# FernandoSchett/parallel_finite_difference_computation

Hardware: AMD Instinct MI355X
Metric: Gpoints/s (stencil updates) + achieved HBM GB/s vs peak (higher is better)
Workload: dtype f32

## Files before the change

include/fdwave.h:

```cpp
#ifndef FDWAVE_H
#define FDWAVE_H

#include <stddef.h>

#ifdef __cplusplus
extern "C" {
#endif

#define FDW_VERSION 2
#define FDW_MAX_ORDER 32

#define FDW_OK 0
#define FDW_EINVAL (-1)
#define FDW_ENODEVICE (-2)
#define FDW_EHIP (-3)
#define FDW_ENOMEM (-4)
#define FDW_ESTATE (-5)
#define FDW_ECOMM (-6)

typedef struct fdw_ctx fdw_ctx;

typedef struct fdw_params {
    int order;
    int nxe, nze;
// ... 212 lines not shown
int fdw_image_unscale_v2(const float *v2, int nxe, int nze, int nxb, int nzb, int nx, int nz, const float *img , float *out);
int fdw_shot_dtt(fdw_ctx *ctx, const float *v2 , int sx, int sz, int gz, const float *srce, const float *d_obs, float *imloc,
                 float *illum , int residual , float *resid , float *P, float *PP);
int fdw_shot_line_dtt(fdw_ctx *ctx, const float *v2, int sz, int gz, const float *wav, const float *d_obs, float *imloc, float *illum, int residual,
                      float *resid, float *P, float *PP);
int fdw_shot_batch_dtt(fdw_ctx *ctx, int nshots, const float *v2_all, unsigned long long draw_offset, int sx0, int dsx, int sz, int gz,
                       const float *srce, const float *d_obs, float *imloc, float *illum, int residual, float *resid);
int fdw_shot_line_batch_dtt(fdw_ctx *ctx, int nshots, const float *v2_all, unsigned long long draw_offset, int sz, int gz, const float *wav_all,
                            const float *d_obs, float *imloc, float *illum, int residual, float *resid);

int fdw_set_tuning(fdw_ctx *ctx, int xchunk, int wz, int use_generic, int prefetch, int two_step);
int fdw_get_tables(const fdw_ctx *ctx, float *coefs_x, float *coefs_z, float *taper_x, float *taper_z);
int fdw_get_extents(const fdw_ctx *ctx, int *xlim, int *zlim, int *ztap);
int fdw_debug_step4_plan(fdw_ctx *ctx, int forward, int sx, int sz, int r0, int r1, int r0b, int r1b, int xchunk, int *nblk, int *nstrip,
                         unsigned char *cls, int cls_cap);
int fdw_two_step_active(const fdw_ctx *ctx);
int fdw_steps_per_pass(const fdw_ctx *ctx);
int fdw_selftest(fdw_ctx *ctx);
int fdw_trace_active(void);

#define FDW_PASS_DEPTH_MAX 3
typedef struct fdw_band_unit {
    int pass, band;
    int r0, r1;
    int stream;
    int nwait;
    int wait[FDW_PASS_DEPTH_MAX - 1];
} fdw_band_unit;
int fdw_plan_pass_bands(int nxl, int upd_x1, int xchunk, int bands, int depth, int npasses, int *bands_out, int *depth_out,
                        fdw_band_unit *units, int cap);
int fdw_set_pass_bands(fdw_ctx *ctx, int bands, int depth);
int fdw_pass_bands(const fdw_ctx *ctx, int *bands, int *depth);

int fdw_calc_coefs(int order, int cxx, float *coef );
void fdw_ricker_wavelet(int nt, float dt, float fpeak, float *s);
void fdw_taper_tables(int nxb, int nzb, float fac, float *taper_x, float *taper_z);
void fdw_extendvel_linear(int nx, int nz, int nxb, int nzb, float *vel);
void fdw_srand(unsigned seed);

#ifdef __cplusplus
}
#endif
#endif
```

parallel_finite_difference_computation_amd/__init__.py:

```python
from ._lib import BORN_DTT, BORN_FIELD, IMAGE_DTT, IMAGE_XCORR, FdwError, LIB_PATH, MODE_FWD, MODE_PLAIN, MODE_RECV, lib
from .api import (FDWave, calc_coefs, extendvel_linear, fd_back, fd_forward, fd_init, image_compare, gather_misfit, gather_scale_v2, image_unscale_v2, image_compensate, image_excitation, image_laplacian, mod_extendvel,
                  mod_ricker_wavelet, mod_taper_tables, ricker_wavelet, snap_dims, srand, taper_tables, planewave_lags, encode_line_source, encode_gathers, encode_gathers_multi, plan_pass_bands)

from .slabs import Comm, Slabs, run_ranks

__all__ = ["Comm", "Slabs", "run_ranks", "FDWave", "FdwError", "calc_coefs", "ricker_wavelet", "taper_tables", "extendvel_linear", "srand",
           "fd_init", "fd_forward", "fd_back", "mod_extendvel", "mod_ricker_wavelet", "mod_taper_tables", "image_laplacian", "image_compare", "image_compensate", "image_excitation", "gather_misfit", "snap_dims", "planewave_lags", "encode_line_source", "encode_gathers", "encode_gathers_multi", "plan_pass_bands", "lib", "LIB_PATH", "MODE_FWD", "MODE_PLAIN", "MODE_RECV", "BORN_FIELD", "BORN_DTT", "IMAGE_XCORR", "IMAGE_DTT", "gather_scale_v2", "image_unscale_v2"]
```

parallel_finite_difference_computation_amd/_lib.py:

```python
import ctypes as C
import os

import numpy as np

_HERE = os.path.dirname(os.path.abspath(__file__))
LIB_PATH = os.environ.get("FDW_LIB") or os.path.join(_HERE, "libfdwave.so")

f32p = np.ctypeslib.ndpointer(dtype=np.float32, flags="C_CONTIGUOUS")
vp = C.c_void_p

FDW_OK, FDW_EINVAL, FDW_ENODEVICE, FDW_EHIP, FDW_ENOMEM, FDW_ESTATE = 0, -1, -2, -3, -4, -5
MODE_FWD, MODE_PLAIN, MODE_RECV = 0, 1, 2
BORN_FIELD, BORN_DTT = 0, 1
IMAGE_XCORR, IMAGE_DTT = 0, 1


class FdwError(RuntimeError):
    def __init__(self, code, msg):
        super().__init__(f"libfdwave error {code}: {msg}")
        self.code = code


class Params(C.Structure):
    _fields_ = [("order", C.c_int), ("nxe", C.c_int), ("nze", C.c_int), ("nxb", C.c_int), ("nzb", C.c_int),
# ... 122 lines not shown
    ("fdw_dev_line_record_illum_steps", C.c_int, [vp, C.POINTER(vp), vp, vp, C.c_int, C.c_int, vp, vp, C.c_int, C.c_int, C.c_int, C.POINTER(C.c_int), C.POINTER(C.c_int), vp]),
    ("fdw_shot_line_residual", C.c_int, [vp, vp, C.c_int, C.c_int, f32p, f32p, f32p, vp, vp, vp, vp]),
    ("fdw_shot_line_batch", C.c_int, [vp, C.c_int, vp, C.c_ulonglong, C.c_int, C.c_int, f32p, f32p, f32p, vp]),
    ("fdw_shot_line_batch_residual", C.c_int, [vp, C.c_int, vp, C.c_ulonglong, C.c_int, C.c_int, f32p, f32p, f32p, vp, vp]),
    ("fdw_record_shot_line_batch", C.c_int, [vp, C.c_int, vp, C.c_ulonglong, C.c_int, C.c_int, f32p, f32p]),
    ("fdw_encode_gathers_multi", C.c_int, [C.c_int, C.c_int, C.c_int, vp, vp, vp, C.c_int, C.c_int, vp]),
    ("fdw_dev_excite_steps", C.c_int, [vp, C.POINTER(vp), vp, vp, C.c_int, C.c_int, vp, vp, C.c_int, C.c_int, C.c_int, C.POINTER(C.c_int), C.POINTER(C.c_int), vp]),
    ("fdw_dev_line_pick_steps", C.c_int, [vp, C.POINTER(vp), vp, vp, C.c_int, vp, C.c_int, vp, C.c_int, C.c_int, C.c_int, C.POINTER(C.c_int), C.POINTER(C.c_int), vp]),
    ("fdw_shot_excitation", C.c_int, [vp, vp, C.c_int, C.c_int, C.c_int, vp, vp, C.c_float, vp, vp, vp, vp, vp, vp]),
    ("fdw_image_excitation", C.c_int, [vp, vp, C.c_size_t, C.c_float, vp]),
    ("fdw_dev_image_excitation", C.c_int, [vp, vp, vp, C.c_float, vp, vp]),
    ("fdw_shot_excitation_batch", C.c_int, [vp, C.c_int, vp, C.c_ulonglong, C.c_int, C.c_int, C.c_int, C.c_int, vp, vp, C.c_float, vp, vp, vp, vp, vp]),
    ("fdw_dev_born_steps", C.c_int, [vp, vp, vp, vp, vp, vp, vp, C.c_int, vp, C.c_int, C.c_int, C.c_int, vp, vp, C.c_int, C.c_int, C.c_int, vp]),
    ("fdw_born_shot", C.c_int, [vp, vp, f32p, C.c_int, C.c_int, C.c_int, C.c_int, f32p, f32p, vp]),
    ("fdw_dev_born_line_steps", C.c_int, [vp, vp, vp, vp, vp, vp, vp, C.c_int, vp, C.c_int, C.c_int, vp, vp, C.c_int, C.c_int, C.c_int, vp]),
    ("fdw_born_shot_line", C.c_int, [vp, vp, vp, C.c_int, C.c_int, C.c_int, vp, vp, vp]),
    ("fdw_born_shot_batch", C.c_int, [vp, C.c_int, vp, C.c_ulonglong, vp, C.c_int, C.c_int, C.c_int, C.c_int, C.c_int, vp, vp, vp]),
    ("fdw_born_shot_line_batch", C.c_int, [vp, C.c_int, vp, C.c_ulonglong, vp, C.c_int, C.c_int, C.c_int, vp, vp, vp]),
    ("fdw_dev_back_iter_dtt", C.c_int, [vp, C.c_int, vp, vp, vp, vp, vp, C.c_int, C.c_int, C.c_int, vp, C.c_int, vp, vp]),
    ("fdw_dev_dtt_image", C.c_int, [vp, vp, vp, vp, vp, vp, vp]),
    ("fdw_gather_scale_v2", C.c_int, [f32p, C.c_int, C.c_int, C.c_int, C.c_int, C.c_int, C.c_int, f32p, f32p]),
    ("fdw_image_unscale_v2", C.c_int, [f32p, C.c_int, C.c_int, C.c_int, C.c_int, C.c_int, C.c_int, f32p, f32p]),
    ("fdw_shot_dtt", C.c_int, [vp, vp, C.c_int, C.c_int, C.c_int, f32p, f32p, f32p, vp, C.c_int, vp, vp, vp]),
    ("fdw_shot_line_dtt", C.c_int, [vp, vp, C.c_int, C.c_int, f32p, f32p, f32p, vp, C.c_int, vp, vp, vp]),
    ("fdw_shot_batch_dtt", C.c_int, [vp, C.c_int, vp, C.c_ulonglong, C.c_int, C.c_int, C.c_int, C.c_int, f32p, f32p, f32p, vp, C.c_int, vp]),
    ("fdw_shot_line_batch_dtt", C.c_int, [vp, C.c_int, vp, C.c_ulonglong, C.c_int, C.c_int, f32p, f32p, f32p, vp, C.c_int, vp]),
    ("fdw_two_step_active", C.c_int, [vp]),
    ("fdw_steps_per_pass", C.c_int, [vp]),
    ("fdw_selftest", C.c_int, [vp]),
    ("fdw_trace_active", C.c_int, []),
    ("fdw_plan_pass_bands", C.c_int, [C.c_int] * 6 + [C.POINTER(C.c_int)] * 2 + [vp, C.c_int]),
    ("fdw_set_pass_bands", C.c_int, [vp, C.c_int, C.c_int]),
    ("fdw_pass_bands", C.c_int, [vp, C.POINTER(C.c_int), C.POINTER(C.c_int)]),
    ("fdw_calc_coefs", C.c_int, [C.c_int, C.c_int, f32p]),
    ("fdw_ricker_wavelet", None, [C.c_int, C.c_float, C.c_float, f32p]),
    ("fdw_taper_tables", None, [C.c_int, C.c_int, C.c_float, vp, vp]),
    ("fdw_extendvel_linear", None, [C.c_int, C.c_int, C.c_int, C.c_int, f32p]),
    ("fdw_srand", None, [C.c_uint]),
]

_lib = None


def lib():
    global _lib
    if _lib is None:
        if not os.path.exists(LIB_PATH):
            raise ImportError(f"{LIB_PATH} is missing: build it with `make -C {os.path.join(_HERE, 'csrc')}` "
                              "(hipcc, gfx950).  There is no CPU fallback.")
        L = C.CDLL(LIB_PATH, mode=C.RTLD_GLOBAL)
        for name, res, args in SIGNATURES:
            fn = getattr(L, name)
            fn.restype = res
            fn.argtypes = args
        _lib = L
    return _lib


def check(rc):
    if rc != 0:
        raise FdwError(rc, lib().fdw_last_error().decode(errors="replace"))
```

parallel_finite_difference_computation_amd/api.py:

```python
import ctypes as C
import sys

import numpy as np

from . import _lib
from ._lib import Params, Slab, Snaps, check, lib


def _f32(a, shape=None):
    a = np.ascontiguousarray(a, dtype=np.float32)
    if shape is not None and a.shape != tuple(shape):
        raise ValueError(f"expected shape {tuple(shape)}, got {a.shape}")
    return a


def calc_coefs(order, cxx=False):
    c = np.zeros(order + 1, np.float32)
    check(lib().fdw_calc_coefs(order, int(cxx), c))
    return c


def ricker_wavelet(nt, dt, fpeak):
    s = np.zeros(nt, np.float32)
    lib().fdw_ricker_wavelet(nt, dt, fpeak, s)
# ... 79 lines not shown

def gather_scale_v2(v2, nxb, gz, g):
    v2, g = np.ascontiguousarray(v2, np.float32), np.ascontiguousarray(g, np.float32)
    out = np.empty_like(g)
    check(lib().fdw_gather_scale_v2(v2, v2.shape[0], v2.shape[1], int(nxb), int(gz), g.shape[0], g.shape[1], g, out))
    return out


def image_unscale_v2(v2, nxb, nzb, img):
    v2, img = np.ascontiguousarray(v2, np.float32), np.ascontiguousarray(img, np.float32)
    out = np.empty_like(img)
    check(lib().fdw_image_unscale_v2(v2, v2.shape[0], v2.shape[1], int(nxb), int(nzb), img.shape[0], img.shape[1], img, out))
    return out


def snap_dims(nx, nz, nt, every, dec=1):
    a, b, c = C.c_int(), C.c_int(), C.c_int()
    check(lib().fdw_snap_dims(nx, nz, nt, int(every), int(dec), C.byref(a), C.byref(b), C.byref(c)))
    return a.value, b.value, c.value


def _i32(a):
    return np.ascontiguousarray(a, dtype=np.int32).reshape(-1)


def plan_pass_bands(nxl, upd_x1, xchunk, bands, depth, npasses):
    g, d = C.c_int(), C.c_int()
    n = lib().fdw_plan_pass_bands(nxl, upd_x1, xchunk, bands, depth, npasses, C.byref(g), C.byref(d), None, 0)
    check(min(n, 0))
    units = (_lib.BandUnit * n)()
    check(min(lib().fdw_plan_pass_bands(nxl, upd_x1, xchunk, bands, depth, npasses, C.byref(g), C.byref(d), units, n), 0))
    return g.value, d.value, [dict(pass_=u.pass_, band=u.band, r0=u.r0, r1=u.r1, stream=u.stream, wait=[u.wait[k] for k in range(u.nwait)])
                              for u in units]


def planewave_lags(src_ix, dx, dt, p):
    src_ix = _i32(src_ix)
    lag = np.zeros(src_ix.size, np.int32)
    check(lib().fdw_planewave_lags(src_ix.size, src_ix.ctypes.data, dx, dt, float(p), lag.ctypes.data))
    return lag


def encode_line_source(src_ix, lag, weight, srce, nx):
    src_ix, lag, weight, srce = _i32(src_ix), _i32(lag), _f32(weight).reshape(-1), _f32(srce).reshape(-1)
    if not (src_ix.size == lag.size == weight.size):
        raise ValueError("src_ix, lag and weight must have one entry per shot")
    wav = np.zeros((nx, srce.size), np.float32)
    check(lib().fdw_encode_line_source(src_ix.size, src_ix.ctypes.data, lag.ctypes.data, weight.ctypes.data, srce.ctypes.data, srce.size, nx,
                                       wav.ctypes.data))
    return wav


def encode_gathers(lag, weight, d_obs_all, device=0):
    lag, weight = _i32(lag), _f32(weight).reshape(-1)
    d_obs_all = np.ascontiguousarray(d_obs_all, np.float32)
    if d_obs_all.ndim != 3 or not (d_obs_all.shape[0] == lag.size == weight.size):
        raise ValueError("d_obs_all must be [nshots][nx][nt] with one lag and one weight per shot")
    _, nx, nt = d_obs_all.shape
    out = np.zeros((nx, nt), np.float32)
    check(lib().fdw_encode_gathers(device, lag.size, lag.ctypes.data, weight.ctypes.data, d_obs_all.ctypes.data, nx, nt, out.ctypes.data))
    return out


def encode_gathers_multi(lag, weight, d_obs_all, device=0):
    lag, weight = np.ascontiguousarray(lag, np.int32), _f32(weight)
    d_obs_all = np.ascontiguousarray(d_obs_all, np.float32)
# ... 36 lines not shown
            self.close()
        except Exception:
            pass

    def tables(self):
        cx = np.zeros(self.order + 1, np.float32)
        cz = np.zeros(self.order + 1, np.float32)
        tx = np.zeros(max(self.nxb, 1), np.float32)
        tz = np.zeros(max(self.nzb, 1), np.float32)
        check(lib().fdw_get_tables(self._h, cx.ctypes.data, cz.ctypes.data, tx.ctypes.data, tz.ctypes.data))
        return cx, cz, tx[:self.nxb], tz[:self.nzb]

    def extents(self):
        a, b, c = C.c_int(), C.c_int(), C.c_int()
        check(lib().fdw_get_extents(self._h, C.byref(a), C.byref(b), C.byref(c)))
        return a.value, b.value, c.value

    def set_tuning(self, xchunk=0, wz=0, use_generic=False, prefetch=0, two_step=0, force_edge=False):
        check(lib().fdw_set_tuning(self._h, xchunk, wz, int(use_generic), prefetch, int(two_step)))

    def two_step_active(self):
        return bool(lib().fdw_two_step_active(self._h))

    def steps_per_pass(self):
        return int(lib().fdw_steps_per_pass(self._h))

    def set_pass_bands(self, bands=0, depth=0):
        check(lib().fdw_set_pass_bands(self._h, int(bands), int(depth)))

    def pass_bands(self):
        a, b = C.c_int(), C.c_int()
        check(lib().fdw_pass_bands(self._h, C.byref(a), C.byref(b)))
        return a.value, b.value

    def selftest(self):
        check(lib().fdw_selftest(self._h))

    def laplacian(self, p):
        p = _f32(p, (self.nxe, self.nze))
        out = np.empty_like(p)
        check(lib().fdw_laplacian(self._h, p, out))
        return out

    def forward(self, v2, sx, sz, srce, p=None, pp=None, nsteps=None):
        shape = (self.nxe, self.nze)
        p = np.zeros(shape, np.float32) if p is None else np.array(p, np.float32, order="C")
        pp = np.zeros(shape, np.float32) if pp is None else np.array(pp, np.float32, order="C")
        srce = _f32(srce)
        nsteps = len(srce) if nsteps is None else nsteps
        if nsteps > len(srce):
            raise ValueError("srce shorter than nsteps")
        check(lib().fdw_forward(self._h, p, pp, _f32(v2, shape), sx, sz, srce, nsteps))
        return p, pp

    def back(self, v2, snap0, snap1, d_obs, gz, imloc=None, nsteps=None):
        shape = (self.nxe, self.nze)
        imloc = np.zeros((self.nx, self.nz), np.float32) if imloc is None else np.array(imloc, np.float32, order="C")
        nsteps = self.nt if nsteps is None else nsteps
        check(lib().fdw_back(self._h, _f32(v2, shape), _f32(snap0, shape), _f32(snap1, shape),
                             _f32(d_obs, (self.nx, self.nt)), gz, imloc, nsteps))
        return imloc

    def shot(self, v2, sx, sz, gz, srce, d_obs, imloc=None, want_fields=False, want_illum=False, illum=None):
        shape = (self.nxe, self.nze)
        imloc = np.zeros((self.nx, self.nz), np.float32) if imloc is None else np.array(imloc, np.float32, order="C")
        P = np.zeros(shape, np.float32) if want_fields else None
# ... 500 lines not shown
```

parallel_finite_difference_computation_amd/csrc/fdw_api.cpp:

```cpp
#include <hip/hip_runtime.h>

#include <algorithm>
#include <climits>
#include <cmath>
#include <cstdarg>
#include <cstdio>
#include <cstdlib>
#include <cstring>
#include <mutex>
#include <new>
#include <type_traits>
#include <vector>

#include "fdw_born.h"
#include "fdw_dtt.h"
#include "fdw_excimg.h"
#include "fdw_internal.h"
#include "fdw_kernels.h"
#include "fdwave.h"

using namespace fdw;

static thread_local char g_err[512] = "";

// ... 54 lines not shown
    int nbatch = 1, batch_dsx = 0, batch_cap = 0, batch_nt = 0;
    bool batch_all = false;
    float* bfld[8] = {nullptr, nullptr, nullptr, nullptr, nullptr, nullptr, nullptr, nullptr};
    float *b_v2 = nullptr, *b_img = nullptr, *b_dobs = nullptr;
    float* b_illum = nullptr;
    int b_illum_cap = 0;
    bool batch_illum = false;
    float* b_rec = nullptr;
    size_t b_rec_cap = 0;
    float* d_wav = nullptr;
    size_t wav_cap = 0;
    float* b_wav = nullptr;
    size_t b_wav_cap = 0;
    float* d_raw = nullptr;
    size_t raw_cap = 0;
    int no_fused_back = 0;
    int no_back_pipe = 0;
    int no_back_fused = 0;
    int no_born_fused = 0;
    float* d_born_m = nullptr;
    float* d_born_rec0 = nullptr;
    size_t born_rec0_cap = 0;
    float* d_dtt_w = nullptr;
    float* d_born_w = nullptr;
    float* b_born_rec0 = nullptr;
    size_t b_born_rec0_cap = 0;
    size_t store_budget = 0;
    int store_segments = 0;
    size_t batch_budget = 0;
    int batch_parts = 0;
    bool batch_single = false;
    int pb_bands = 0, pb_depth = 0;
    int pb_used_bands = 0, pb_used_depth = 0;
    hipStream_t pb_side[FDW_PASS_DEPTH_MAX - 1] = {};
    hipEvent_t pb_fork = nullptr, pb_join[FDW_PASS_DEPTH_MAX - 1] = {}, pb_ring[kBandRing] = {};
};

static size_t field_elems(const fdw_ctx* c) { return (size_t)c->nxl * (size_t)c->pitch; }

extern "C" int fdw_pitch(const fdw_ctx* c) { return c ? c->pitch : 0; }
extern "C" size_t fdw_field_bytes(const fdw_ctx* c) { return c ? field_elems(c) * sizeof(float) : 0; }

static int is_full_grid(const fdw_ctx* c) { return c->slab.x_off == 0 && c->nxl == c->prm.nxe; }

static hipStream_t pick_stream(fdw_ctx* c, void* s) { return s ? (hipStream_t)s : c->stream; }

static int alloc_zero(float** p, size_t elems)
{
    if (*p) return FDW_OK;
    hipError_t e = hipMalloc((void**)p, elems * sizeof(float));
    if (e != hipSuccess) return fail(FDW_ENOMEM, "hipMalloc(%zu bytes) failed: %s", elems * sizeof(float), hipGetErrorString(e));
    HIP_TRY(hipMemset(*p, 0, elems * sizeof(float)));
    HIP_TRY(hipDeviceSynchronize());
    return FDW_OK;
}

static int ensure_work_buffers(fdw_ctx* c, int nfields, bool need_img)
{
    for (int i = 0; i < nfields; i++) {
        int rc = alloc_zero(&c->fld[i], field_elems(c));
        if (rc) return rc;
    }
    int rc = alloc_zero(&c->d_v2, field_elems(c));
    if (rc) return rc;
    if (need_img) {
        rc = alloc_zero(&c->d_img, field_elems(c));
// ... 710 lines not shown
    if (c->tb == kPipeSteps) return true;
    if (c->tb > 0) return false;
    return (long)c->upd_x1 * ((c->pitch / 4 + 55) / 56) >= kPipeAutoStripRows;
}

struct StepnBack {
    float *lvl0 = nullptr, *lvl1 = nullptr;
    const float* plev[kPipeSteps] = {};
    float* img = nullptr;
    int inj_stride = 0;
    const float *rp = nullptr, *rpp = nullptr;
    float *rout1 = nullptr, *rout2 = nullptr;
};
static void tile_classes(const Step2Args& a, const FwdVariant& v, std::vector<unsigned char>& cls)
{
    constexpr int H = kMaxFastHalfOrder, NS = kPipeSteps;
    cls.resize((size_t)a.nblk);
    for (int L = 0; L < a.nblk; L++) {
        FDW_PIPE_TILE_ROWS(a, L, zb, xa, xe)
        const int cs = FDW_PIPE_TILE_CELL(zb, NS);
        const bool lean = v.kmode == FDW_MODE_PLAIN ? pipe_tile_lean<H, NS, false, 0>(a, cs, xa, xe)
                          : (v.line && v.rec)       ? pipe_tile_lean<H, NS, true, 2, false, true>(a, cs, xa, xe)
                          : v.line                  ? pipe_tile_lean<H, NS, true, 2>(a, cs, xa, xe)
                                                    : pipe_tile_lean<H, NS, true, 1>(a, cs, xa, xe);
        cls[(size_t)L] = lean ? 0 : 1;
    }
}

static int pipe_strips(const fdw_ctx* c)
{
    const int ncells = c->pitch / 4, own = 64 - 2 * kPipeSteps;
    return (ncells + own - 1) / own;
}
static int pipe_fwd_xchunk(const fdw_ctx* c, long strip_rows)
{
    const bool fastnum = c->prm.numerics == FDW_NUMERICS_FAST;
    return c->xchunk2 > 0 ? c->xchunk2 : (strip_rows >= 1000000 ? 253 : (strip_rows >= 250000 ? 173 : (strip_rows >= 120000 ? (fastnum ? 173 : 143) : (strip_rows >= 60000 ? 83 : 43))));
}

struct StepnPlan {
    int nblk = 0, nstrip = 0;
    std::vector<unsigned char> cls;
};
static thread_local StepnPlan* g_plan = nullptr;

static int stepn_impl(fdw_ctx* c, int mode, const float* d_p, const float* d_pp, const float* d_v2, float* d_out1, float* d_out2, int pp_twice,
                      const FwdView& f, const StepnBack& bk, const RowRanges& rr, hipStream_t s)
{
    const bool recv = mode == FDW_MODE_RECV || mode == FDW_MODE_BACK4;
    if (c->h != kMaxFastHalfOrder) return fail(FDW_EINVAL, "stepn: the pipelined kernel is built for order 8 only");
    if (mode != FDW_MODE_FWD && mode != FDW_MODE_PLAIN && mode != FDW_MODE_MOD && mode != FDW_MODE_PLAIN_ALL && mode != FDW_MODE_RECV && mode != FDW_MODE_BACK4)
        return fail(FDW_EINVAL, "stepn: FWD, PLAIN, PLAIN_ALL, RECV, BACK4 or MOD only");
    if (mode == FDW_MODE_BACK4) {
        if (!bk.img || !f.samples || !bk.rp || !bk.rpp || !bk.rout1 || !bk.rout2) return fail(FDW_EINVAL, "stepn: BACK4 needs the receiver pair, its outputs, samples and image");
        const float* all[8] = {d_p, d_pp, d_out1, d_out2, bk.rp, bk.rpp, bk.rout1, bk.rout2};
        for (int i = 0; i < 8; i++)
            for (int j = i + 1; j < 8; j++)
                if (all[i] == all[j]) return fail(FDW_EINVAL, "stepn: BACK4 buffers must not alias");
    }
    if ((mode == FDW_MODE_PLAIN_ALL && (!bk.lvl0 || !bk.lvl1)) ||
        (mode == FDW_MODE_RECV && (!bk.img || !f.samples || !bk.plev[0] || !bk.plev[1] || !bk.plev[2] || !bk.plev[3])))
        return fail(FDW_EINVAL, "stepn: the backward passes need their level buffers / source fields, samples and image");
    if ((mode == FDW_MODE_MOD) != (c->prm.dialect == FDW_DIALECT_MOD)) return fail(FDW_ESTATE, "stepn: mode %d does not belong to dialect %d", mode, c->prm.dialect);
    if (!d_p || !d_pp || !d_v2 || !d_out1 || !d_out2) return fail(FDW_EINVAL, "stepn: NULL buffer");
    if (d_out1 == d_p || d_out1 == d_pp || d_out2 == d_p || d_out2 == d_pp || d_out1 == d_out2)
        return fail(FDW_EINVAL, "stepn: outputs must not alias the inputs (tiles re-read each other's input rows)");
    Step2Args a{};
    fill_common(c, a, d_p, d_pp, d_v2, pp_twice);
    a.out1 = d_out1; a.out2 = d_out2;
// ... 172 lines not shown
    if (npasses > INT_MAX / G) return fail(FDW_EINVAL, "pass bands: %d passes of %d bands", npasses, G);
    if (bands_out) *bands_out = G;
    if (depth_out) *depth_out = D;
    const int total = G * npasses;
    for (int i = 0; units && i < std::min(cap, total); i++) {
        fdw_band_unit& u = units[i];
        u.pass = i / G; u.band = i % G;
        u.r0 = G == 1 ? 0 : first_chunk(u.band) * xchunk;
        u.r1 = u.band == G - 1 ? nxl : first_chunk(u.band + 1) * xchunk;
        u.stream = i % D;
        u.nwait = 0;
        for (int k = 0; k < FDW_PASS_DEPTH_MAX - 1; k++) u.wait[k] = -1;
        for (int j = i - D - 1; j >= i - 2 * D + 1 && j >= 0; j--) u.wait[u.nwait++] = j;
    }
    return total;
}

extern "C" int fdw_set_pass_bands(fdw_ctx* c, int bands, int depth)
{
    if (!c) return fail(FDW_EINVAL, "ctx is NULL");
    if (bands < 0 || depth < 0 || depth > FDW_PASS_DEPTH_MAX || (bands == 0) != (depth == 0))
        return fail(FDW_EINVAL, "pass bands: bands=%d depth=%d (0, 0 = automatic; depth 1..%d)", bands, depth, FDW_PASS_DEPTH_MAX);
    c->pb_bands = bands; c->pb_depth = depth;
    return FDW_OK;
}

extern "C" int fdw_pass_bands(const fdw_ctx* c, int* bands, int* depth)
{
    if (!c || !bands || !depth) return fail(FDW_EINVAL, "NULL argument");
    *bands = c->pb_used_bands; *depth = c->pb_used_depth;
    return FDW_OK;
}

constexpr int kBandAutoTiles = 1776, kBandAutoPasses = 8;
static void wanted_pass_bands(const fdw_ctx* c, long tiles, int npasses, int* bands, int* depth)
{
    *bands = *depth = 1;
    if (c->pb_bands > 0) {
        *bands = c->pb_bands; *depth = c->pb_depth;
    } else if (const char* e = getenv("FDW_PASS_BANDS")) {
        int g = 0, d = 0;
        if (sscanf(e, "%d,%d", &g, &d) == 2 && g >= 1 && d >= 1 && d <= FDW_PASS_DEPTH_MAX) { *bands = g; *depth = d; }
    } else if (tiles >= kBandAutoTiles && npasses >= kBandAutoPasses) {
        *bands = 3; *depth = 2;
    }
}

static int ensure_band_streams(fdw_ctx* c, int depth)
{
    if (!c->pb_fork) HIP_TRY(hipEventCreateWithFlags(&c->pb_fork, hipEventDisableTiming));
    for (hipEvent_t& e : c->pb_ring)
        if (!e) HIP_TRY(hipEventCreateWithFlags(&e, hipEventDisableTiming));
    for (int j = 0; j < depth - 1; j++) {
        if (!c->pb_side[j]) HIP_TRY(hipStreamCreateWithFlags(&c->pb_side[j], hipStreamNonBlocking));
        if (!c->pb_join[j]) HIP_TRY(hipEventCreateWithFlags(&c->pb_join[j], hipEventDisableTiming));
    }
    return FDW_OK;
}

static int band_passes(fdw_ctx* c, float* const* buf, const float* d_v2, const Forward& f, int it0, int npasses, int first_pp_twice, int* ip, int* ipp,
                       hipStream_t s, int G, int D, int xchunk)
{
    std::vector<fdw_band_unit> units((size_t)G * npasses);
    int g_ = 0, d_ = 0;
    const int total = fdw_plan_pass_bands(c->nxl, c->upd_x1, xchunk, G, D, npasses, &g_, &d_, units.data(), (int)units.size());
    if (total < 0) return total;
    if (g_ != G || d_ != D || total != (int)units.size()) return fail(FDW_ESTATE, "pass bands: the plan changed between two calls");
    hipStream_t st[FDW_PASS_DEPTH_MAX] = {s};
    if (D > 1) {
        FDW_TRY(ensure_band_streams(c, D));
        HIP_TRY(hipEventRecord(c->pb_fork, s));
        for (int j = 1; j < D; j++) {
            st[j] = c->pb_side[j - 1];
            HIP_TRY(hipStreamWaitEvent(st[j], c->pb_fork, 0));
        }
    }
    auto issue = [&]() -> int {
        int o1 = 0, o2 = 0;
        for (int i = 0; i < total; i++) {
            const fdw_band_unit& u = units[(size_t)i];
            if (u.band == 0) spare_pair(*ip, *ipp, &o1, &o2);
            const int k = u.pass * kPipeSteps;
            for (int w = 0; w < u.nwait; w++) HIP_TRY(hipStreamWaitEvent(st[u.stream], c->pb_ring[u.wait[w] % kBandRing], 0));
            FDW_TRY(stepn_impl(c, FDW_MODE_FWD, buf[*ipp], buf[*ip], d_v2, buf[o1], buf[o2], (k > 0) || first_pp_twice, view_at(f, it0 + k, c->nx), StepnBack{},
                                RowRanges{u.r0, u.r1, 0, 0, xchunk}, st[u.stream]));
            if (D > 1 && i + D + 1 < total) HIP_TRY(hipEventRecord(c->pb_ring[i % kBandRing], st[u.stream]));
            if (u.band == G - 1) { *ip = o1; *ipp = o2; }
        }
        return FDW_OK;
    };
    const int rc = issue();
    char msg[sizeof g_err];
    if (rc != FDW_OK) memcpy(msg, g_err, sizeof msg);
    int jrc = FDW_OK;
    for (int j = 1; j < D; j++) {
        hipError_t e = hipEventRecord(c->pb_join[j - 1], st[j]);
        if (e == hipSuccess) e = hipStreamWaitEvent(s, c->pb_join[j - 1], 0);
        if (e != hipSuccess && jrc == FDW_OK) jrc = fail(FDW_EHIP, "pass bands: joining side stream %d failed: %s", j, hipGetErrorString(e));
    }
    if (rc != FDW_OK) memcpy(g_err, msg, sizeof msg);
    return rc != FDW_OK ? rc : jrc;
}

static int single_steps_on_copies(fdw_ctx* c, float* const* buf, const float* d_v2, const Forward& f, int it, int m, int twice, int ip, int ipp, int o1,
                                  int o2, hipStream_t s)
{
    const size_t bytes = field_elems(c) * sizeof(float) * (size_t)std::max(c->nbatch, 1);
    const float* newest = buf[ipp];
    for (int j = 0; j < m; j++) {
        float* dst = buf[(j & 1) ? o2 : o1];
        if (j < 2) HIP_TRY(hipMemcpyAsync(dst, buf[j == 0 ? ip : ipp], bytes, hipMemcpyDeviceToDevice, s));
        FDW_TRY(step_impl(c, FDW_MODE_FWD, newest, dst, d_v2, 0, c->nxl, twice || j > 0, view_at(f, it + j, c->nx), BackExtra{}, s));
        newest = dst;
    }
    return FDW_OK;
}

static int steps_loop(fdw_ctx* c, float* const* buf, const float* d_v2, const Forward& f, int it0, int nsteps, int first_pp_twice, int* ip, int* ipp,
                      hipStream_t s)
{
    if (!c || !buf || !ip || !ipp) return fail(FDW_EINVAL, "NULL argument");
    if (*ip < 0 || *ip > 3 || *ipp < 0 || *ipp > 3 || *ip == *ipp) return fail(FDW_EINVAL, "steps2: bad buffer indices");
    const FwdVariant var = fwd_variant(FDW_MODE_FWD, f);
    if (var.kmode < 0) return fail(FDW_EINVAL, "steps: no kernel is built for this combination of a line source, recording, illumination and excitation");
    if (f.rec) FDW_TRY(record_static(c, buf[*ip], buf[*ipp], f.gz, f.rec, it0, nsteps, s));
    int k = 0;
    c->pb_used_bands = c->pb_used_depth = 1;
    if (f.may_band && var.kmode == FDW_MODE_FWD && c->nbatch <= 1 && nsteps >= kPipeSteps && pipe_pays(c)) {
        const int nstrip = pipe_strips(c), xchunk = pipe_fwd_xchunk(c, (long)c->upd_x1 * nstrip), npasses = nsteps / kPipeSteps;
        int G, D;
        wanted_pass_bands(c, (long)nstrip * ((c->upd_x1 + xchunk - 1) / xchunk), npasses, &G, &D);
        if (G > 1 && fdw_plan_pass_bands(c->nxl, c->upd_x1, xchunk, G, D, npasses, &G, &D, nullptr, 0) < 0) return FDW_EINVAL;
        if (G > 1) {
            c->pb_used_bands = G; c->pb_used_depth = D;
            FDW_TRY(band_passes(c, buf, d_v2, f, it0, npasses, first_pp_twice, ip, ipp, s, G, D, xchunk));
            k = npasses * kPipeSteps;
        }
    }
    while (k < nsteps) {
        const int twice = (k > 0) || first_pp_twice;
        const FwdView v = view_at(f, it0 + k, c->nx);
        const int m = (nsteps - k >= kPipeSteps && pipe_pays(c)) ? kPipeSteps : ((nsteps - k >= 2 && two_step_pays(c)) ? 2 : 1);
        if (m == 1) {
            std::swap(*ip, *ipp);
            FDW_TRY(step_impl(c, FDW_MODE_FWD, buf[*ip], buf[*ipp], d_v2, 0, c->nxl, twice, v, BackExtra{}, s));
            k += 1;
            continue;
        }
        int o1, o2;
        spare_pair(*ip, *ipp, &o1, &o2);
        if (!family_serves(m, var))
            FDW_TRY(single_steps_on_copies(c, buf, d_v2, f, it0 + k, m, twice, *ip, *ipp, o1, o2, s));
        else if (m == kPipeSteps)
            FDW_TRY(stepn_impl(c, FDW_MODE_FWD, buf[*ipp], buf[*ip], d_v2, buf[o1], buf[o2], twice, v, StepnBack{}, RowRanges{}, s));
        else
            FDW_TRY(step2_impl(c, FDW_MODE_FWD, buf[*ipp], buf[*ip], d_v2, buf[o1], buf[o2], twice, v, BackExtra{}, s));
        *ip = o1; *ipp = o2;
        k += m;
    }
    return FDW_OK;
}

extern "C" int fdw_dev_steps2(fdw_ctx* c, float* const* buf, const float* d_v2, const float* d_srce, int sx, int sz, int it0, int nsteps,
                              int first_pp_twice, int* ip, int* ipp, void* stream)
{
// ... 2176 lines not shown
```

Before: 721.0.

## Add moving-cut two-stream pass schedule for temporally blocked forward steps

Adds a pass scheduler that splits each multi-step pass at a cut column which sweeps back and forth between lo and hi chunks. The two halves run on two streams with event waits only where halo reach overlaps, so consecutive passes can overlap and tail underutilisation is hidden. A three-piece turn handles direction reversals, and medium-sized grids get a different x-chunk size (213). The band executor is generalised into unit_passes, which records events only for units that are actually awaited. The cost is more event and stream synchronisation and a more complex dependency plan.

```diff
diff --git a/include/fdwave.h b/include/fdwave.h
--- a/include/fdwave.h
+++ b/include/fdwave.h
@@ -268,6 +268,11 @@
 int fdw_set_pass_bands(fdw_ctx *ctx, int bands, int depth);
 int fdw_pass_bands(const fdw_ctx *ctx, int *bands, int *depth);
 
+int fdw_plan_pass_cut(int nxl, int upd_x1, int xchunk, int cut_lo, int cut_hi, int npasses, int *lo_out, int *hi_out, fdw_band_unit *units,
+                      int cap);
+int fdw_set_pass_cut(fdw_ctx *ctx, int lo, int hi);
+int fdw_pass_cut(const fdw_ctx *ctx, int *lo, int *hi, int *turns);
+
 int fdw_calc_coefs(int order, int cxx, float *coef );
 void fdw_ricker_wavelet(int nt, float dt, float fpeak, float *s);
 void fdw_taper_tables(int nxb, int nzb, float fac, float *taper_x, float *taper_z);
diff --git a/parallel_finite_difference_computation_amd/__init__.py b/parallel_finite_difference_computation_amd/__init__.py
--- a/parallel_finite_difference_computation_amd/__init__.py
+++ b/parallel_finite_difference_computation_amd/__init__.py
@@ -1,8 +1,8 @@
 from ._lib import BORN_DTT, BORN_FIELD, IMAGE_DTT, IMAGE_XCORR, FdwError, LIB_PATH, MODE_FWD, MODE_PLAIN, MODE_RECV, lib
 from .api import (FDWave, calc_coefs, extendvel_linear, fd_back, fd_forward, fd_init, image_compare, gather_misfit, gather_scale_v2, image_unscale_v2, image_compensate, image_excitation, image_laplacian, mod_extendvel,
-                  mod_ricker_wavelet, mod_taper_tables, ricker_wavelet, snap_dims, srand, taper_tables, planewave_lags, encode_line_source, encode_gathers, encode_gathers_multi, plan_pass_bands)
+                  mod_ricker_wavelet, mod_taper_tables, ricker_wavelet, snap_dims, srand, taper_tables, planewave_lags, encode_line_source, encode_gathers, encode_gathers_multi, plan_pass_bands, plan_pass_cut)
 
 from .slabs import Comm, Slabs, run_ranks
 
 __all__ = ["Comm", "Slabs", "run_ranks", "FDWave", "FdwError", "calc_coefs", "ricker_wavelet", "taper_tables", "extendvel_linear", "srand",
-           "fd_init", "fd_forward", "fd_back", "mod_extendvel", "mod_ricker_wavelet", "mod_taper_tables", "image_laplacian", "image_compare", "image_compensate", "image_excitation", "gather_misfit", "snap_dims", "planewave_lags", "encode_line_source", "encode_gathers", "encode_gathers_multi", "plan_pass_bands", "lib", "LIB_PATH", "MODE_FWD", "MODE_PLAIN", "MODE_RECV", "BORN_FIELD", "BORN_DTT", "IMAGE_XCORR", "IMAGE_DTT", "gather_scale_v2", "image_unscale_v2"]
+           "fd_init", "fd_forward", "fd_back", "mod_extendvel", "mod_ricker_wavelet", "mod_taper_tables", "image_laplacian", "image_compare", "image_compensate", "image_excitation", "gather_misfit", "snap_dims", "planewave_lags", "encode_line_source", "encode_gathers", "encode_gathers_multi", "plan_pass_bands", "plan_pass_cut", "lib", "LIB_PATH", "MODE_FWD", "MODE_PLAIN", "MODE_RECV", "BORN_FIELD", "BORN_DTT", "IMAGE_XCORR", "IMAGE_DTT", "gather_scale_v2", "image_unscale_v2"]
diff --git a/parallel_finite_difference_computation_amd/_lib.py b/parallel_finite_difference_computation_amd/_lib.py
--- a/parallel_finite_difference_computation_amd/_lib.py
+++ b/parallel_finite_difference_computation_amd/_lib.py
@@ -178,6 +178,9 @@
     ("fdw_plan_pass_bands", C.c_int, [C.c_int] * 6 + [C.POINTER(C.c_int)] * 2 + [vp, C.c_int]),
     ("fdw_set_pass_bands", C.c_int, [vp, C.c_int, C.c_int]),
     ("fdw_pass_bands", C.c_int, [vp, C.POINTER(C.c_int), C.POINTER(C.c_int)]),
+    ("fdw_plan_pass_cut", C.c_int, [C.c_int] * 6 + [C.POINTER(C.c_int)] * 2 + [vp, C.c_int]),
+    ("fdw_set_pass_cut", C.c_int, [vp, C.c_int, C.c_int]),
+    ("fdw_pass_cut", C.c_int, [vp] + [C.POINTER(C.c_int)] * 3),
     ("fdw_calc_coefs", C.c_int, [C.c_int, C.c_int, f32p]),
     ("fdw_ricker_wavelet", None, [C.c_int, C.c_float, C.c_float, f32p]),
     ("fdw_taper_tables", None, [C.c_int, C.c_int, C.c_float, vp, vp]),
diff --git a/parallel_finite_difference_computation_amd/api.py b/parallel_finite_difference_computation_amd/api.py
--- a/parallel_finite_difference_computation_amd/api.py
+++ b/parallel_finite_difference_computation_amd/api.py
@@ -135,6 +135,16 @@
     check(min(lib().fdw_plan_pass_bands(nxl, upd_x1, xchunk, bands, depth, npasses, C.byref(g), C.byref(d), units, n), 0))
     return g.value, d.value, [dict(pass_=u.pass_, band=u.band, r0=u.r0, r1=u.r1, stream=u.stream, wait=[u.wait[k] for k in range(u.nwait)])
                               for u in units]
+
+
+def plan_pass_cut(nxl, upd_x1, xchunk, cut_lo, cut_hi, npasses):
+    lo, hi = C.c_int(), C.c_int()
+    n = lib().fdw_plan_pass_cut(nxl, upd_x1, xchunk, cut_lo, cut_hi, npasses, C.byref(lo), C.byref(hi), None, 0)
+    check(min(n, 0))
+    units = (_lib.BandUnit * n)()
+    check(min(lib().fdw_plan_pass_cut(nxl, upd_x1, xchunk, cut_lo, cut_hi, npasses, C.byref(lo), C.byref(hi), units, n), 0))
+    return lo.value, hi.value, [dict(pass_=u.pass_, band=u.band, r0=u.r0, r1=u.r1, stream=u.stream, wait=[u.wait[k] for k in range(u.nwait)])
+                                for u in units]
 
 
 def planewave_lags(src_ix, dx, dt, p):
@@ -237,6 +247,14 @@
         a, b = C.c_int(), C.c_int()
         check(lib().fdw_pass_bands(self._h, C.byref(a), C.byref(b)))
         return a.value, b.value
+
+    def set_pass_cut(self, lo=0, hi=0):
+        check(lib().fdw_set_pass_cut(self._h, int(lo), int(hi)))
+
+    def pass_cut(self):
+        a, b, t = C.c_int(), C.c_int(), C.c_int()
+        check(lib().fdw_pass_cut(self._h, C.byref(a), C.byref(b), C.byref(t)))
+        return a.value, b.value, t.value
 
     def selftest(self):
         check(lib().fdw_selftest(self._h))
diff --git a/parallel_finite_difference_computation_amd/csrc/fdw_api.cpp b/parallel_finite_difference_computation_amd/csrc/fdw_api.cpp
--- a/parallel_finite_difference_computation_amd/csrc/fdw_api.cpp
+++ b/parallel_finite_difference_computation_amd/csrc/fdw_api.cpp
@@ -110,6 +110,8 @@
     bool batch_single = false;
     int pb_bands = 0, pb_depth = 0;
     int pb_used_bands = 0, pb_used_depth = 0;
+    int pc_lo = 0, pc_hi = 0;
+    int pc_used_lo = -1, pc_used_hi = -1, pc_used_turns = 0;
     hipStream_t pb_side[FDW_PASS_DEPTH_MAX - 1] = {};
     hipEvent_t pb_fork = nullptr, pb_join[FDW_PASS_DEPTH_MAX - 1] = {}, pb_ring[kBandRing] = {};
 };
@@ -886,9 +888,13 @@
     const int ncells = c->pitch / 4, own = 64 - 2 * kPipeSteps;
     return (ncells + own - 1) / own;
 }
-static int pipe_fwd_xchunk(const fdw_ctx* c, long strip_rows)
+static int pipe_fwd_xchunk(const fdw_ctx* c, long strip_rows, bool moving_cut = false)
 {
     const bool fastnum = c->prm.numerics == FDW_NUMERICS_FAST;
+    if (c->xchunk2 <= 0) {
+        if (const char* e = getenv("FDW_FWD_XCHUNK")) if (atoi(e) > 0) return atoi(e);
+        if (moving_cut && strip_rows >= 250000 && strip_rows < 1000000) return 213;
+    }
     return c->xchunk2 > 0 ? c->xchunk2 : (strip_rows >= 1000000 ? 253 : (strip_rows >= 250000 ? 173 : (strip_rows >= 120000 ? (fastnum ? 173 : 143) : (strip_rows >= 60000 ? 83 : 43))));
 }
 
@@ -1127,6 +1133,93 @@
     return FDW_OK;
 }
 
+extern "C" int fdw_plan_pass_cut(int nxl, int upd_x1, int xchunk, int cut_lo, int cut_hi, int npasses, int* lo_out, int* hi_out,
+                                 fdw_band_unit* units, int cap)
+{
+    if (nxl <= 0 || upd_x1 < 0 || upd_x1 > nxl || xchunk <= 0 || cut_lo < 0 || cut_hi < cut_lo || npasses < 1 || (units && cap < 0))
+        return fail(FDW_EINVAL, "pass cut: nxl=%d upd_x1=%d xchunk=%d cut=[%d,%d] npasses=%d", nxl, upd_x1, xchunk, cut_lo, cut_hi, npasses);
+    constexpr int reach = kPipeSteps * kMaxFastHalfOrder;
+    const int nchunks = (upd_x1 + xchunk - 1) / xchunk;
+    const bool safe = xchunk >= reach && nchunks >= 3 && cut_lo < cut_hi && cut_lo >= 1 && cut_hi < nchunks && upd_x1 - (long)cut_hi * xchunk >= reach;
+    if (npasses > INT_MAX / 3) return fail(FDW_EINVAL, "pass cut: %d passes", npasses);
+    if (lo_out) *lo_out = safe ? cut_lo : 0;
+    if (hi_out) *hi_out = safe ? cut_hi : 0;
+    auto clear_waits = [](fdw_band_unit& u) {
+        u.nwait = 0;
+        for (int k = 0; k < FDW_PASS_DEPTH_MAX - 1; k++) u.wait[k] = -1;
+    };
+    if (!safe) {
+        for (int i = 0; units && i < std::min(cap, npasses); i++) {
+            fdw_band_unit& u = units[i];
+            u.pass = i; u.band = 0; u.r0 = 0; u.r1 = nxl; u.stream = 0;
+            clear_waits(u);
+        }
+        return npasses;
+    }
+    auto meet = [](int a0, int a1, int b0, int b1) { return a0 < b1 && b0 < a1; };
+    int total = 0;
+    fdw_band_unit prev{};
+    auto emit = [&](int pass, int band, int r0, int r1) {
+        const int i = total++;
+        fdw_band_unit u{};
+        u.pass = pass; u.band = band; u.r0 = r0; u.r1 = r1;
+        u.stream = i % 2;
+        clear_waits(u);
+        if (i >= 1 && prev.pass != pass) {
+            const int rd0 = std::max(r0 - reach, 0), rd1 = std::min(r1 + reach, nxl);
+            const int prd0 = std::max(prev.r0 - reach, 0), prd1 = std::min(prev.r1 + reach, nxl);
+            if (meet(prev.r0, prev.r1, rd0, rd1) || meet(r0, r1, prd0, prd1)) u.wait[u.nwait++] = i - 1;
+        }
+        if (i >= 3) u.wait[u.nwait++] = i - 3;
+        if (units && i < cap) units[i] = u;
+        prev = u;
+    };
+    const bool three = cut_hi - cut_lo >= 4;
+    const int X = xchunk;
+    int cut = cut_hi, dir = -1;
+    for (int n = 0; n < npasses; n++) {
+        if (n > 0 && three && dir < 0 && cut == cut_lo + 1) {
+            emit(n, 0, 0, cut_lo * X);
+            emit(n, 1, (cut_lo + 2) * X, nxl);
+            emit(n, 2, cut_lo * X, (cut_lo + 2) * X);
+            cut = cut_lo + 2; dir = 1;
+            continue;
+        }
+        if (n > 0 && three && dir > 0 && cut == cut_hi - 1) {
+            emit(n, 1, cut_hi * X, nxl);
+            emit(n, 0, 0, (cut_hi - 2) * X);
+            emit(n, 2, (cut_hi - 2) * X, cut_hi * X);
+            cut = cut_hi - 2; dir = -1;
+            continue;
+        }
+        if (n > 0) {
+            if (!three && (cut + dir < cut_lo || cut + dir > cut_hi)) dir = -dir;
+            cut += dir;
+        }
+        for (int k = 0; k < 2; k++) {
+            if ((k == 0) == (dir < 0)) emit(n, 0, 0, cut * X);
+            else emit(n, 1, cut * X, nxl);
+        }
+    }
+    return total;
+}
+
+extern "C" int fdw_set_pass_cut(fdw_ctx* c, int lo, int hi)
+{
+    if (!c) return fail(FDW_EINVAL, "ctx is NULL");
+    if (!((lo == 0 && hi == 0) || (lo == -1 && hi == -1) || (lo >= 1 && hi >= lo)))
+        return fail(FDW_EINVAL, "pass cut: lo=%d hi=%d (0, 0 = automatic; -1, -1 = off; else 1 <= lo <= hi)", lo, hi);
+    c->pc_lo = lo; c->pc_hi = hi;
+    return FDW_OK;
+}
+
+extern "C" int fdw_pass_cut(const fdw_ctx* c, int* lo, int* hi, int* turns)
+{
+    if (!c || !lo || !hi || !turns) return fail(FDW_EINVAL, "NULL argument");
+    *lo = c->pc_used_lo; *hi = c->pc_used_hi; *turns = c->pc_used_turns;
+    return FDW_OK;
+}
+
 constexpr int kBandAutoTiles = 1776, kBandAutoPasses = 8;
 static void wanted_pass_bands(const fdw_ctx* c, long tiles, int npasses, int* bands, int* depth)
 {
@@ -1141,6 +1234,22 @@
     }
 }
 
+constexpr long kCutAutoMinStripRows = 60000, kCutAutoMaxStripRows = 500000;
+static bool wanted_pass_cut(const fdw_ctx* c, long strip_rows, int nchunks, int npasses, int* lo, int* hi)
+{
+    if (c->pc_lo >= 1) { *lo = c->pc_lo; *hi = c->pc_hi; return true; }
+    if (c->pc_lo < 0) return false;
+    if (const char* e = getenv("FDW_PASS_CUT")) {
+        int a = 0, b = 0;
+        if (sscanf(e, "%d,%d", &a, &b) != 2 || a < 1 || b < a) return false;
+        *lo = a; *hi = b;
+        return true;
+    }
+    if (strip_rows < kCutAutoMinStripRows || strip_rows >= kCutAutoMaxStripRows || npasses < kBandAutoPasses) return false;
+    *lo = nchunks / 3; *hi = nchunks - nchunks / 3;
+    return true;
+}
+
 static int ensure_band_streams(fdw_ctx* c, int depth)
 {
     if (!c->pb_fork) HIP_TRY(hipEventCreateWithFlags(&c->pb_fork, hipEventDisableTiming));
@@ -1153,14 +1262,19 @@
     return FDW_OK;
 }
 
-static int band_passes(fdw_ctx* c, float* const* buf, const float* d_v2, const Forward& f, int it0, int npasses, int first_pp_twice, int* ip, int* ipp,
-                       hipStream_t s, int G, int D, int xchunk)
-{
-    std::vector<fdw_band_unit> units((size_t)G * npasses);
-    int g_ = 0, d_ = 0;
-    const int total = fdw_plan_pass_bands(c->nxl, c->upd_x1, xchunk, G, D, npasses, &g_, &d_, units.data(), (int)units.size());
-    if (total < 0) return total;
-    if (g_ != G || d_ != D || total != (int)units.size()) return fail(FDW_ESTATE, "pass bands: the plan changed between two calls");
+static int unit_passes(fdw_ctx* c, float* const* buf, const float* d_v2, const Forward& f, int it0, int first_pp_twice, int* ip, int* ipp, hipStream_t s,
+                       const std::vector<fdw_band_unit>& units, int D, int xchunk)
+{
+    const int total = (int)units.size();
+    std::vector<char> awaited((size_t)total, 0);
+    for (int i = 0; i < total; i++) {
+        const fdw_band_unit& u = units[(size_t)i];
+        if (u.stream < 0 || u.stream >= D || u.nwait < 0 || u.nwait > FDW_PASS_DEPTH_MAX - 1) return fail(FDW_ESTATE, "pass units: unit %d is malformed", i);
+        for (int w = 0; w < u.nwait; w++) {
+            if (u.wait[w] < 0 || u.wait[w] >= i || i - u.wait[w] >= kBandRing) return fail(FDW_ESTATE, "pass units: unit %d waits for unit %d", i, u.wait[w]);
+            awaited[(size_t)u.wait[w]] = 1;
+        }
+    }
     hipStream_t st[FDW_PASS_DEPTH_MAX] = {s};
     if (D > 1) {
         FDW_TRY(ensure_band_streams(c, D));
@@ -1174,13 +1288,13 @@
         int o1 = 0, o2 = 0;
         for (int i = 0; i < total; i++) {
             const fdw_band_unit& u = units[(size_t)i];
-            if (u.band == 0) spare_pair(*ip, *ipp, &o1, &o2);
+            if (i == 0 || units[(size_t)i - 1].pass != u.pass) spare_pair(*ip, *ipp, &o1, &o2);
             const int k = u.pass * kPipeSteps;
             for (int w = 0; w < u.nwait; w++) HIP_TRY(hipStreamWaitEvent(st[u.stream], c->pb_ring[u.wait[w] % kBandRing], 0));
             FDW_TRY(stepn_impl(c, FDW_MODE_FWD, buf[*ipp], buf[*ip], d_v2, buf[o1], buf[o2], (k > 0) || first_pp_twice, view_at(f, it0 + k, c->nx), StepnBack{},
                                 RowRanges{u.r0, u.r1, 0, 0, xchunk}, st[u.stream]));
-            if (D > 1 && i + D + 1 < total) HIP_TRY(hipEventRecord(c->pb_ring[i % kBandRing], st[u.stream]));
-            if (u.band == G - 1) { *ip = o1; *ipp = o2; }
+            if (D > 1 && awaited[(size_t)i]) HIP_TRY(hipEventRecord(c->pb_ring[i % kBandRing], st[u.stream]));
+            if (i + 1 == total || units[(size_t)i + 1].pass != u.pass) { *ip = o1; *ipp = o2; }
         }
         return FDW_OK;
     };
@@ -1197,6 +1311,31 @@
     return rc != FDW_OK ? rc : jrc;
 }
 
+static int band_passes(fdw_ctx* c, float* const* buf, const float* d_v2, const Forward& f, int it0, int npasses, int first_pp_twice, int* ip, int* ipp,
+                       hipStream_t s, int G, int D, int xchunk)
+{
+    std::vector<fdw_band_unit> units((size_t)G * npasses);
+    int g_ = 0, d_ = 0;
+    const int total = fdw_plan_pass_bands(c->nxl, c->upd_x1, xchunk, G, D, npasses, &g_, &d_, units.data(), (int)units.size());
+    if (total < 0) return total;
+    if (g_ != G || d_ != D || total != (int)units.size()) return fail(FDW_ESTATE, "pass bands: the plan changed between two calls");
+    return unit_passes(c, buf, d_v2, f, it0, first_pp_twice, ip, ipp, s, units, D, xchunk);
+}
+
+static int cut_passes(fdw_ctx* c, float* const* buf, const float* d_v2, const Forward& f, int it0, int npasses, int first_pp_twice, int* ip, int* ipp,
+                      hipStream_t s, int lo, int hi, int xchunk, int* turns)
+{
+    int lo_ = 0, hi_ = 0;
+    const int total = fdw_plan_pass_cut(c->nxl, c->upd_x1, xchunk, lo, hi, npasses, &lo_, &hi_, nullptr, 0);
+    if (total < 0) return total;
+    std::vector<fdw_band_unit> units((size_t)total);
+    if (lo_ != lo || hi_ != hi || fdw_plan_pass_cut(c->nxl, c->upd_x1, xchunk, lo, hi, npasses, &lo_, &hi_, units.data(), total) != total)
+        return fail(FDW_ESTATE, "pass cut: the plan changed between two calls");
+    *turns = 0;
+    for (int i = 1; i < total; i++) *turns += units[(size_t)i].band == 2 || (units[(size_t)i].nwait > 0 && units[(size_t)i].wait[0] == i - 1);
+    return unit_passes(c, buf, d_v2, f, it0, first_pp_twice, ip, ipp, s, units, 2, xchunk);
+}
+
 static int single_steps_on_copies(fdw_ctx* c, float* const* buf, const float* d_v2, const Forward& f, int it, int m, int twice, int ip, int ipp, int o1,
                                   int o2, hipStream_t s)
 {
@@ -1221,11 +1360,25 @@
     if (f.rec) FDW_TRY(record_static(c, buf[*ip], buf[*ipp], f.gz, f.rec, it0, nsteps, s));
     int k = 0;
     c->pb_used_bands = c->pb_used_depth = 1;
+    c->pc_used_lo = c->pc_used_hi = -1; c->pc_used_turns = 0;
     if (f.may_band && var.kmode == FDW_MODE_FWD && c->nbatch <= 1 && nsteps >= kPipeSteps && pipe_pays(c)) {
-        const int nstrip = pipe_strips(c), xchunk = pipe_fwd_xchunk(c, (long)c->upd_x1 * nstrip), npasses = nsteps / kPipeSteps;
-        int G, D;
-        wanted_pass_bands(c, (long)nstrip * ((c->upd_x1 + xchunk - 1) / xchunk), npasses, &G, &D);
-        if (G > 1 && fdw_plan_pass_bands(c->nxl, c->upd_x1, xchunk, G, D, npasses, &G, &D, nullptr, 0) < 0) return FDW_EINVAL;
+        const int nstrip = pipe_strips(c), npasses = nsteps / kPipeSteps;
+        const long strip_rows = (long)c->upd_x1 * nstrip;
+        const int xchunk = pipe_fwd_xchunk(c, strip_rows), xcut = pipe_fwd_xchunk(c, strip_rows, true);
+        int G = 1, D = 1, lo = 0, hi = 0;
+        const bool bands_set = c->pb_bands > 0 || getenv("FDW_PASS_BANDS");
+        if (!bands_set && wanted_pass_cut(c, strip_rows, (c->upd_x1 + xcut - 1) / xcut, npasses, &lo, &hi)) {
+            if (fdw_plan_pass_cut(c->nxl, c->upd_x1, xcut, lo, hi, npasses, &lo, &hi, nullptr, 0) < 0) return FDW_EINVAL;
+            if (lo > 0) {
+                c->pb_used_bands = c->pb_used_depth = 2;
+                c->pc_used_lo = lo; c->pc_used_hi = hi;
+                FDW_TRY(cut_passes(c, buf, d_v2, f, it0, npasses, first_pp_twice, ip, ipp, s, lo, hi, xcut, &c->pc_used_turns));
+                k = npasses * kPipeSteps;
+            }
+        } else {
+            wanted_pass_bands(c, (long)nstrip * ((c->upd_x1 + xchunk - 1) / xchunk), npasses, &G, &D);
+            if (G > 1 && fdw_plan_pass_bands(c->nxl, c->upd_x1, xchunk, G, D, npasses, &G, &D, nullptr, 0) < 0) return FDW_EINVAL;
+        }
         if (G > 1) {
             c->pb_used_bands = G; c->pb_used_depth = D;
             FDW_TRY(band_passes(c, buf, d_v2, f, it0, npasses, first_pp_twice, ip, ipp, s, G, D, xchunk));
```

Result: faster. 738.9, median of 6 (+2.5%).
